# zbw2577/fea-large

Measured on AMD Instinct MI355X. Metric: element-stiffness assemblies/sec, higher is better.
Workload: dtype f64; 1 GPU; 10349856 TET4/1GP neohookean block (66x396x66 Kuhn cubes on the 1x6x1 bar), stiffness+residual assembly, deformed state k1=1.1; elements=10349856, nodes=1782133, scalar_nnz=236453589, clock_ramp_launches_before_warmup=80

## Files before the change

fea-large_amd/csrc/feahip_internal.h:

```cpp
#pragma once
#include <hip/hip_runtime.h>
#include <algorithm>
#include <cstdint>
#include <cstdio>
#include <functional>
#include <initializer_list>
#include <string>
#include <thread>
#include <type_traits>
#include <vector>
#include "../../include/fea_hip.h"

hipError_t feahip_device_malloc(void **p, size_t bytes);
#define hipMalloc(p, bytes) feahip_device_malloc((void **)(p), (bytes))

#define FEA_MAX_NPE 10
#define FEA_MAX_GAUSS 27

#define FEA_CHUNK_BLOCKS 128
#define FEA_CHUNK_ROWS 16
#define FEA_WAVES_PER_WG 4
#define FEA_RED_BLOCKS 2048

struct ElemTable {
// ... 202 lines not shown
#ifndef FEA_Q_SLOTS
#define FEA_Q_SLOTS 5
#endif
#define FEA_Q_REGW 4
#define FEA_Q_MAX_PASS 7
#define FEA_Q_FLANES 128
#define FEA_Q_ROWS_U16 200
struct Gather10Header {
  int r0, r1, b0, nb;
  int nnode, nelem, ntask, npass;
  int nft, fdw;
  unsigned char prow[8];
  unsigned char cnt[40];
  unsigned char sw[8];
  int pad[8];
};
static_assert(FEA_Q_SLOTS * FEA_Q_WAVES <= 40 && FEA_Q_SLOTS <= 8, "Gather10Header: cnt / sw too small");
static_assert(sizeof(Gather10Header) == 128, "Gather10Header is 128 bytes");
struct Gather10Layout {
  int stride;
  int o_nodes, o_elems, o_rows, o_tpos, o_flist, o_clist;
  int max_nodes, max_elems, max_cw, max_fdw, tile_blocks;
};
enum Gather10Limit {
  G10_FITS = FEAHIP_G10_LIMIT_NONE, G10_ELEMS = FEAHIP_G10_LIMIT_ELEMS, G10_ROW_LENGTH = FEAHIP_G10_LIMIT_ROW_LENGTH,
  G10_TASKS = FEAHIP_G10_LIMIT_TASKS, G10_RESIDUAL_LANES = FEAHIP_G10_LIMIT_RESIDUAL_LANES,
  G10_LIST_LENGTH = FEAHIP_G10_LIMIT_LIST_LENGTH, G10_PASSES = FEAHIP_G10_LIMIT_PASSES, G10_OTHER = FEAHIP_G10_LIMIT_OTHER
};
struct HostGather10 : HostChunkMaps {
  Gather10Layout lay;
  std::vector<int> elist;
  int npe = 10;
  int limit = G10_FITS;
  int limit_row = -1;
  int tile_blocks = 0;
};
void build_host_gather10(int N, int E, int npe, const int *conn, const HostPattern &hp, int row_lo, int row_hi, HostGather10 &out);
int ensure_gather10(feahip_ctx *c);
int launch_assemble_gather10(feahip_ctx *c, bool doK, bool doF);

int launch_assemble_visit(feahip_ctx *c, bool doK, bool doF);

enum class MapOutcome { none, built, failed, declined };
struct MapCache {
  int key0 = -1, key1 = -1;
  MapOutcome outcome = MapOutcome::none;
  long long bytes = 0;
  bool built() const { return outcome == MapOutcome::built; }
  bool is(MapOutcome o, int k0, int k1) const { return outcome == o && key0 == k0 && key1 == k1; }
  bool settled(int k0, int k1) const { return is(MapOutcome::built, k0, k1) || is(MapOutcome::failed, k0, k1); }
  void record(MapOutcome o, int k0, int k1) { outcome = o; key0 = k0; key1 = k1; }
};
inline void dev_free(std::initializer_list<void *> ptrs) { for (void *p : ptrs) if (p) (void)hipFree(p); }
struct GenericMaps : MapCache {
  int *d_incptr = nullptr;
  uint32_t *d_inc = nullptr;
  uint8_t *d_incslot = nullptr;
  void release() { dev_free({d_incptr, d_inc, d_incslot}); *this = GenericMaps(); }
};
struct VisitMaps : MapCache {
  VisitDesc *d_desc = nullptr;
  int *d_node = nullptr;
  uint32_t *d_rec = nullptr;
  int nrecords = 0;
  void release() { dev_free({d_desc, d_node, d_rec}); *this = VisitMaps(); }
};
struct QuadMaps : MapCache {
  QuadDesc *d_desc = nullptr;
  uint32_t *d_elem = nullptr, *d_pair = nullptr;
  int *d_node = nullptr;
  int nchunks = 0;
  void release() { dev_free({d_desc, d_elem, d_pair, d_node}); *this = QuadMaps(); }
};
struct GatherCache : MapCache {
  unsigned char *d_maps = nullptr;
  int nchunks = 0;
  double evals_per_element = 0;
  int same_words = 0;
};
struct GatherMaps : GatherCache {
  GatherLayout lay{};
  int *d_run_start = nullptr;
  int nruns = 0;
  std::vector<int> record_of;
  void release() { dev_free({d_maps, d_run_start}); *this = GatherMaps(); }
};
struct Gather10Maps : GatherCache {
  Gather10Layout lay{};
  int *d_elist = nullptr;
  double *d_state = nullptr;
  int nloc = 0;
  void release() { dev_free({d_maps, d_elist, d_state}); *this = Gather10Maps(); }
};

struct SurfaceLoads {
  int nfaces = 0, npf = 0;
  std::vector<int> h_lnode;
  int *d_fnode = nullptr;
  int *d_kind = nullptr;
  double *d_val = nullptr;
  double *d_fc = nullptr;
  int *d_lnode = nullptr, *d_lptr = nullptr, *d_lslot = nullptr;
  void release() { dev_free({d_fnode, d_kind, d_val, d_fc, d_lnode, d_lptr, d_lslot}); *this = SurfaceLoads(); }
};

#define FEA_SURF_MAX_PTS 6
#define FEA_SURF_MAX_NPF 6
struct FaceRule {
  int npt;
  double w[FEA_SURF_MAX_PTS];
  double N[FEA_SURF_MAX_PTS][FEA_SURF_MAX_NPF];
  double dN[FEA_SURF_MAX_PTS][2][FEA_SURF_MAX_NPF];
};
void face_rule(int npf, FaceRule &R);

struct ContactObstacles {
  int n;
  int kind[FEAHIP_MAX_OBSTACLES];
  double c[FEAHIP_MAX_OBSTACLES][3];
  double a[FEAHIP_MAX_OBSTACLES][3];
  double r[FEAHIP_MAX_OBSTACLES];
};
struct ContactState {
  bool set = false;
  int n = 0, nobs = 0;
  double penalty = 0, gap_tolerance = 0;
  int augment_max = 0;
  int kind[FEAHIP_MAX_OBSTACLES] = {0};
  double geom[FEAHIP_MAX_OBSTACLES][10] = {{0}};
  std::vector<int> h_node;
  std::vector<double> h_w;
  int *d_node = nullptr;
  double *d_w = nullptr;
  double *d_mu = nullptr;
  double *d_part = nullptr;
  void release() { dev_free({d_node, d_w, d_mu, d_part}); *this = ContactState(); }
};

struct MassState {
  bool set = false;
  bool stale = false;
  int n_rho = 0, n_mat = 0, Gm = 0;
  std::vector<double> rho, w, N, dN;
  double *d_m_base = nullptr;
  double *d_m = nullptr;
  long long kb0 = -1, kb1 = -1;
  double *d_vel = nullptr, *d_acc = nullptr, *d_xt = nullptr, *d_vt = nullptr;
  double *d_body = nullptr;
  double body[3] = {0, 0, 0};
  double time = 0;
  double *d_ml = nullptr;
  int ml_row0 = -1, ml_row1 = -1;
  double *d_ke_part = nullptr;
  int ke_parts = 0;
  void release_m() { dev_free({d_m_base}); d_m_base = d_m = nullptr; kb0 = kb1 = -1; }
  void release_lump() { dev_free({d_ml, d_ke_part}); d_ml = d_ke_part = nullptr; ml_row0 = ml_row1 = -1; ke_parts = 0; }
  void release() { dev_free({d_m_base, d_vel, d_acc, d_xt, d_vt, d_body, d_ml, d_ke_part}); *this = MassState(); }
};

struct DampingState {
  double alpha = 0, beta = 0;
  double *d_Kd_alloc = nullptr;
  double *d_Kd_base = nullptr;
  double *d_Kd = nullptr;
  int row0 = -1, row1 = -1;
  bool on() const { return alpha > 0.0 || beta > 0.0; }
// ... 525 lines not shown
```

fea-large_amd/csrc/gather_device.h:

```cpp
#pragma once
#include "fem_device.h"
#define PRIO_STATE 0
#define PRIO_GATHER 1
#define PRIO_OUT 3
#include <algorithm>
#include <cstdlib>
#include <cstring>

struct GatherArgs {
  int chunk0, nchunks, model;
  double lambda, mu;
  const ElemTable *tab;
  const unsigned char *maps;
  GatherLayout lay;
  const double *X0, *x;
  double *K, *f;
  int *bad;
  unsigned long long *stamps;
  int ablate;
  const double2 *mat;
};
#if defined(FEAHIP_DEBUG) && !defined(FEAHIP_NOABL)
#define G_ABL(bit) (A.ablate & (bit))
#else
#define G_ABL(bit) 0
#endif

#ifdef FEAHIP_DEBUG
#define G_STAMP(i) do { if (A.stamps) st[i] = __builtin_amdgcn_s_memtime(); } while (0)
#else
#define G_STAMP(i) do { } while (0)
#endif

#define G_RS 0
#define G_RD 66
#define G_VF 130
#define G_SLOT(w) ((w) & 1023u)
#define G_LA(w) (((w) >> 10) & 3)
#define G_LB(w) (((w) >> 12) & 3)

#define GREC 26
#define GREC_F 12

struct GRead { double2 pa, za, pb, qb, zb, vv; };
__device__ __forceinline__ GRead g_fetch(const double *sT, unsigned w)
{
  const double2 *T = reinterpret_cast<const double2 *>(sT + G_SLOT(w) * GREC);
  const int la = G_LA(w), lb = G_LB(w);
  GRead r;
  r.pa = T[la]; r.za = T[8 + la]; r.pb = T[lb]; r.qb = T[4 + lb]; r.zb = T[8 + lb]; r.vv = T[12];
  return r;
}
__device__ __forceinline__ void g_apply(const GRead &r, double (&acc)[9], double &accd)
{
  const double ga0 = r.pa.x, ga1 = r.pa.y, ga2 = r.za.x;
  const double gb0 = r.pb.x, gb1 = r.pb.y, gb2 = r.zb.x;
  const double tb0 = r.qb.x, tb1 = r.qb.y, tb2 = r.zb.y;
  const double vl = r.vv.x, vm = r.vv.y;
  const double h0 = vl * gb0, h1 = vl * gb1, h2 = vl * gb2;
  const double m0 = vm * gb0, m1 = vm * gb1, m2 = vm * gb2;
  accd = fma(ga0, tb0, fma(ga1, tb1, fma(ga2, tb2, accd)));
  acc[0] = fma(ga0, h0, fma(ga0, m0, acc[0])); acc[1] = fma(ga0, h1, fma(ga1, m0, acc[1])); acc[2] = fma(ga0, h2, fma(ga2, m0, acc[2]));
  acc[3] = fma(ga1, h0, fma(ga0, m1, acc[3])); acc[4] = fma(ga1, h1, fma(ga1, m1, acc[4])); acc[5] = fma(ga1, h2, fma(ga2, m1, acc[5]));
  acc[6] = fma(ga2, h0, fma(ga0, m2, acc[6])); acc[7] = fma(ga2, h1, fma(ga1, m2, acc[7])); acc[8] = fma(ga2, h2, fma(ga2, m2, acc[8]));
}
__device__ __forceinline__ void g_finish(double (&acc)[9], double accd)
{
  acc[0] += accd; acc[4] += accd; acc[8] += accd;
}
__device__ __forceinline__ void g_consume(const double *sT, unsigned w, double (&acc)[9], double &accd)
{
  g_apply(g_fetch(sT, w), acc, accd);
}
__device__ __forceinline__ void g_apply_cheap(const GRead &r, double (&acc)[9])
{
  acc[0] += r.pa.x; acc[1] += r.za.x; acc[2] += r.pb.x; acc[3] += r.qb.x; acc[4] += r.zb.x; acc[5] += r.vv.x;
}
__device__ __forceinline__ GRead g_fetch_cheap(const double *sT, unsigned w)
{
  GRead r; const double v = (double)w;
  r.pa = make_double2(v, v); r.za = r.pa; r.pb = r.pa; r.qb = r.pa; r.zb = r.pa; r.vv = r.pa;
  return r;
}
// ... 181 lines not shown
    for (int b = 0; b < 4; ++b)
#pragma unroll
      for (int i = 0; i < 3; ++i) R[b * 3 + i] = g[b][i];
    const double T00 = S[0][0] + vm, T11 = S[1][1] + vm, T22 = S[2][2] + vm;
#pragma unroll
    for (int b = 0; b < 4; ++b) {
      R[12 + b * 3 + 0] = fma(T00, g[b][0], fma(S[0][1], g[b][1], S[0][2] * g[b][2]));
      R[12 + b * 3 + 1] = fma(T11, g[b][1], fma(S[0][1], g[b][0], S[1][2] * g[b][2]));
      R[12 + b * 3 + 2] = fma(T22, g[b][2], fma(S[0][2], g[b][0], S[1][2] * g[b][1]));
    }
    R[24] = vd * lambda;
    R[25] = vm;
  } else {
#pragma unroll
    for (int b = 1; b < 4; ++b)
#pragma unroll
      for (int i = 0; i < 3; ++i) R[b * 3 + i] = S[i][0] * g[b][0] + S[i][1] * g[b][1] + S[i][2] * g[b][2];
#pragma unroll
    for (int i = 0; i < 3; ++i) R[i] = -((R[3 + i] + R[6 + i]) + R[9 + i]);
  }
  return detJ;
}

template <int CTRL>
__device__ __forceinline__ double g_quad_perm(double x)
{
  int lo = __double2loint(x), hi = __double2hiint(x);
  lo = __builtin_amdgcn_update_dpp(0, lo, CTRL, 0xF, 0xF, true);
  hi = __builtin_amdgcn_update_dpp(0, hi, CTRL, 0xF, 0xF, true);
  return __hiloint2double(hi, lo);
}
__device__ __forceinline__ double g_quad_sum(double v)
{
  v += g_quad_perm<0xB1>(v);
  v += g_quad_perm<0x4E>(v);
  return v;
}

#define G_BARRIER() do { __builtin_amdgcn_fence(__ATOMIC_RELEASE, "workgroup", "local"); __builtin_amdgcn_s_barrier(); \
                         __builtin_amdgcn_fence(__ATOMIC_ACQUIRE, "workgroup", "local"); } while (0)

typedef int g_v8i __attribute__((ext_vector_type(8)));
typedef int g_v4i __attribute__((ext_vector_type(4)));

struct GMaps {
  unsigned eids, tpos, cw[FEA_G_REGW], vw[2];
  int kd, vb, ve;
};

#define G_TASK_THREADS FEA_G_TASK_THREADS

template <bool DOK, bool DOF>
__device__ __forceinline__ void g_load_maps(const GatherLayout &lay, const unsigned char *rec, int t, GMaps &m)
{
  const unsigned short *rows = reinterpret_cast<const unsigned short *>(rec + lay.o_rows);
  m.eids = 0xFFFFFFFFu; m.tpos = 0; m.kd = m.vb = m.ve = 0;
#pragma unroll
  for (int k = 0; k < FEA_G_REGW; ++k) m.cw[k] = 0;
  m.vw[0] = m.vw[1] = 0;
  if (t < lay.max_elems) m.eids = reinterpret_cast<const unsigned *>(rec + lay.o_elems)[t];
  if (DOK && t < ((lay.max_tasks + 63) & ~63)) {
    m.tpos = reinterpret_cast<const unsigned *>(rec + lay.o_bpos)[t];
#pragma unroll
    for (int k = 0; k < FEA_G_REGW; ++k)
      if (k < lay.max_depth) m.cw[k] = reinterpret_cast<const unsigned *>(rec + lay.o_clist)[k * FEA_G_THREADS + t];
  }
  if (DOK && t >= G_TASK_THREADS) {
    const int l = t - G_TASK_THREADS;
    m.kd = rows[G_RD + (l >> 2)];
#pragma unroll
    for (int k = 0; k < FEA_G_REGW; ++k)
      if (k < lay.max_ddepth) m.cw[k] = reinterpret_cast<const unsigned *>(rec + lay.o_dlist)[k * FEA_G_DIAG_LANES + l];
  }
  if (!DOK && t < ((lay.max_vthr + 63) & ~63)) {
#pragma unroll
    for (int v = 0; v < 2; ++v)
      if (v < lay.max_vdepth) m.vw[v] = reinterpret_cast<const unsigned short *>(rec + lay.o_vlist)[v * FEA_G_THREADS + t];
  }
  if (!DOK) {
    const int fr = min(t / 3, FEA_G_MAX_ROWS - 1);
    m.vb = rows[G_VF + fr]; m.ve = rows[G_VF + fr + 1];
  }
}
```

fea-large_amd/csrc/kernels_gather.hip:

```cpp
#include "gather_device.h"
#ifndef G_NT_ROWS
#define G_NT_ROWS 1
#endif
template <bool DOK, bool DOF, bool NH, bool HET>
__global__ __launch_bounds__(FEA_G_THREADS, FEA_G_BIG ? 4 : 3)
void k_assemble_gather(GatherArgs A, const int *__restrict__ run_start, int nruns)
{
  extern __shared__ double2 g_smem[];
  double2 *sC = g_smem;
  double *sT = reinterpret_cast<double *>(g_smem + A.lay.max_nodes * 3);
  const int t = threadIdx.x;
#ifdef FEAHIP_DEBUG
  unsigned long long st[8] = {0, 0, 0, 0, 0, 0, 0, 0}, sa[8] = {0, 0, 0, 0, 0, 0, 0, 0};
  const unsigned long long clk0 = __builtin_amdgcn_s_memtime(), real0 = __builtin_amdgcn_s_memrealtime();
#endif
  const int per = ((int)gridDim.x + 7) >> 3;
  const int ridx = ((int)blockIdx.x & 7) * per + ((int)blockIdx.x >> 3);
  if (ridx >= nruns) return;
  int chunk = run_start[ridx];
  const int cend = run_start[ridx + 1];
  if (chunk >= cend) return;
  constexpr int REC = DOK ? GREC : GREC_F;
  const size_t stride = (size_t)A.lay.stride;
  const unsigned char *rec = A.maps + (size_t)(A.chunk0 + chunk) * stride;
  const bool node_lane = t < A.lay.max_nodes;
  const int wslot = __builtin_amdgcn_readfirstlane(t >> 6);

  const double gauss_w = A.tab->w[0];
  GMaps mn;
  g_load_maps<DOK, DOF>(A.lay, G_ABL(64) ? A.maps + (size_t)A.chunk0 * stride : rec, t, mn);
  GatherHeader hn = *reinterpret_cast<const GatherHeader *>(rec);
  int node1 = reinterpret_cast<const int *>(rec + A.lay.o_nodes)[t & (FEA_G_MAX_NODES - 1)];
  if (node_lane) {
    const double *gx = A.x + (size_t)node1 * 4, *gX = A.X0 + (size_t)node1 * 4;
    const double2 a0 = *reinterpret_cast<const double2 *>(gx), a1 = *reinterpret_cast<const double2 *>(gx + 2);
    const double2 c0 = *reinterpret_cast<const double2 *>(gX), c1 = *reinterpret_cast<const double2 *>(gX + 2);
    sC[t * 3] = a0; sC[t * 3 + 1] = make_double2(a1.x, c0.x); sC[t * 3 + 2] = make_double2(c0.y, c1.x);
  }
  {
    const int cn = min(chunk + 1, cend - 1);
    node1 = reinterpret_cast<const int *>(A.maps + (size_t)(A.chunk0 + cn) * stride + A.lay.o_nodes)[t & (FEA_G_MAX_NODES - 1)];
  }
  int mid1 = 0;
  double2 pn = make_double2(A.lambda, A.mu);
  if constexpr (HET) {
    pn = A.mat[rec[A.lay.o_emat + t]];
    const int cn = min(chunk + 1, cend - 1);
    mid1 = (A.maps + (size_t)(A.chunk0 + cn) * stride + A.lay.o_emat)[t];
    asm volatile("" : : "v"(mid1), "v"(pn.x), "v"(pn.y));
  }
  asm volatile("" : : "v"(mn.eids), "v"(mn.tpos), "v"(mn.cw[0]), "v"(mn.cw[1]), "v"(mn.cw[2]), "v"(mn.cw[3]), "v"(mn.cw[4]), "v"(mn.cw[5]),
               "v"(mn.vw[0]), "v"(mn.vw[1]), "v"(mn.kd), "v"(mn.vb), "v"(mn.ve), "v"(node1), "v"(gauss_w));
  G_BARRIER();

  for (;;) {
    G_STAMP(0);
    const bool more = chunk + 1 < cend;
    const GatherHeader h = hn;
    int hword;
    double2 ca0, ca1, cc0, cc1;
    const GMaps m = mn;
    const int nrows = h.r1 - h.r0;
    const unsigned wdw = wslot < 4 ? h.wdepth[0] : (wslot < 8 ? h.wdepth[1] : h.wdepth[2]);
    const int wd = wslot < G_TASK_THREADS / 64 ? (int)((wdw >> (8 * (wslot & 3))) & 255u) : 0;
    rec = A.maps + (size_t)(A.chunk0 + chunk) * stride;

    __builtin_amdgcn_s_setprio(PRIO_STATE);
    if (t < h.nelem && m.eids != 0xFFFFFFFFu) {
      const unsigned eids = m.eids;
      const int nd[4] = {(int)(eids & 255u), (int)((eids >> 8) & 255u), (int)((eids >> 16) & 255u), (int)(eids >> 24)};
      double xe[4][3], Xe[4][3];
#pragma unroll
      for (int k = 0; k < 4; ++k) {
        const double2 *cc = sC + nd[k] * 3;
        const double2 p0 = cc[0], p1 = cc[1], p2 = cc[2];
        xe[k][0] = p0.x; xe[k][1] = p0.y; xe[k][2] = p1.x;
        Xe[k][0] = p1.y; Xe[k][1] = p2.x; Xe[k][2] = p2.y;
      }
      double R[REC];
      double detJ;
      if (G_ABL(8)) { detJ = 1.0; for (int q = 0; q < REC; ++q) R[q] = xe[q & 3][q % 3] + Xe[(q >> 2) & 3][q % 3]; }
      else detJ = NH ? lintet_record_nh<DOK>(xe, Xe, gauss_w, HET ? pn.x : A.lambda, HET ? pn.y : A.mu, R)
                     : lintet_record_a5<DOK>(xe, Xe, gauss_w, HET ? pn.x : A.lambda, HET ? pn.y : A.mu, R);
      if (!(detJ > 0.0)) {
        if (DOK) {
          const int *gn = reinterpret_cast<const int *>(rec + A.lay.o_nodes);
          const int g0 = min(min(gn[nd[0]], gn[nd[1]]), min(gn[nd[2]], gn[nd[3]]));
          if (g0 >= h.r0 && g0 < h.r1) atomicAdd(A.bad, 1);
        }
      }
      if (detJ == 0.0) {
        double2 *o = reinterpret_cast<double2 *>(sT + t * REC);
#pragma unroll
        for (int q = 0; q < REC / 2; ++q) o[q] = make_double2(0.0, 0.0);
      } else if (!G_ABL(1)) g_store_record<DOK>(sT + t * REC, R);
      else sT[t * REC] = R[0] + R[25 % REC];
    } else if (t < h.nelem) {
      double2 *o = reinterpret_cast<double2 *>(sT + t * REC);
#pragma unroll
      for (int q = 0; q < REC / 2; ++q) o[q] = make_double2(0.0, 0.0);
    }
    {
      const int c1 = min(chunk + 1, cend - 1), c2 = min(chunk + 2, cend - 1);
      const unsigned char *rec1 = A.maps + (size_t)(A.chunk0 + c1) * stride;
      hword = reinterpret_cast<const int *>(rec1)[t & 15];
      if (!(h.flags & 1) || G_ABL(64)) g_load_maps<DOK, DOF>(A.lay, G_ABL(64) ? A.maps + (size_t)A.chunk0 * stride : rec1, t, mn);
      if (wslot < FEA_G_MAX_NODES / 64) {
        const size_t n1 = (size_t)(node_lane ? node1 : 0);
        ca0 = *reinterpret_cast<const double2 *>(A.x + n1 * 4); ca1.x = A.x[n1 * 4 + 2];
        cc0 = *reinterpret_cast<const double2 *>(A.X0 + n1 * 4); cc1.x = A.X0[n1 * 4 + 2];
        node1 = reinterpret_cast<const int *>(A.maps + (size_t)(A.chunk0 + c2) * stride + A.lay.o_nodes)[t & (FEA_G_MAX_NODES - 1)];
      }
      if constexpr (HET) {
        if (wslot * 64 < A.lay.max_elems) {
          pn = A.mat[mid1];
          mid1 = (A.maps + (size_t)(A.chunk0 + c2) * stride + A.lay.o_emat)[t];
        }
      }
    }

    G_LDS_DRAIN();
    G_BARRIER();
    G_STAMP(1);

    __builtin_amdgcn_s_setprio(PRIO_GATHER);
    double acc[9] = {0, 0, 0, 0, 0, 0, 0, 0, 0}, accd = 0;
    if (DOK && t < h.noffd) {
#define G_FETCH(w) (G_ABL(4) ? g_fetch_cheap(sT, w) : g_fetch(sT, w))
#define G_APPLY(r) do { if (G_ABL(2)) g_apply_cheap(r, acc); else g_apply(r, acc, accd); } while (0)
#pragma unroll
      for (int k = 0; k < FEA_G_REGW; ++k)
        if (k < wd) { { const GRead r = G_FETCH(m.cw[k] & 0xFFFFu); G_APPLY(r); } { const GRead r = G_FETCH(m.cw[k] >> 16); G_APPLY(r); } }
      for (int k = FEA_G_REGW; k < wd; ++k) {
        const unsigned w = reinterpret_cast<const unsigned *>(rec + A.lay.o_clist)[k * FEA_G_THREADS + t];
        g_consume(sT, w & 0xFFFFu, acc, accd); g_consume(sT, w >> 16, acc, accd);
      }
      g_finish(acc, accd);
    }
    double dg[6] = {0, 0, 0, 0, 0, 0};
    double fa[3] = {0, 0, 0};
    if (DOK && t >= G_TASK_THREADS && t - G_TASK_THREADS < 4 * nrows) {
#pragma unroll
      for (int k = 0; k < FEA_G_REGW; ++k)
        if (k < h.ddepth) { g_consume_diag<DOF>(sT, m.cw[k] & 0xFFFFu, dg, fa); g_consume_diag<DOF>(sT, m.cw[k] >> 16, dg, fa); }
      for (int k = FEA_G_REGW; k < h.ddepth; ++k) {
        const unsigned w = reinterpret_cast<const unsigned *>(rec + A.lay.o_dlist)[k * FEA_G_DIAG_LANES + t - G_TASK_THREADS];
        g_consume_diag<DOF>(sT, w & 0xFFFFu, dg, fa); g_consume_diag<DOF>(sT, w >> 16, dg, fa);
      }
    }
    if (!DOK && t < h.nvthr) {
      g_visit<DOK>(sT, m.vw[0], fa);
      if (h.vdepth > 1) g_visit<DOK>(sT, m.vw[1], fa);
      for (int v = 2; v < h.vdepth; ++v)
        g_visit<DOK>(sT, reinterpret_cast<const unsigned short *>(rec + A.lay.o_vlist)[v * FEA_G_THREADS + t], fa);
    }
    G_STAMP(2);
    __builtin_amdgcn_s_setprio(PRIO_OUT);
    G_BARRIER();
    G_STAMP(3);

    const int odd = h.b0 & 1;
    double *sK = sT + odd;
    double *sF = DOK ? sT + ((A.lay.max_tile * 9 + 3) & ~1) : sT;
    if (DOK && t < h.noffd && !G_ABL(16)) {
      const int bpos = (int)(m.tpos & 0xFFFFu), mpos = (int)(m.tpos >> 16);
      if (bpos != 0xFFFF) {
#pragma unroll
        for (int q = 0; q < 9; ++q) sK[bpos * 9 + q] = acc[q];
      }
      if (mpos != 0xFFFF) {
#pragma unroll
        for (int i = 0; i < 3; ++i)
#pragma unroll
          for (int j = 0; j < 3; ++j) sK[mpos * 9 + 3 * j + i] = acc[3 * i + j];
      }
    }
    if (DOK && t >= G_TASK_THREADS) {
#pragma unroll
      for (int q = 0; q < 6; ++q) dg[q] = g_quad_sum(dg[q]);
      if (DOF) {
#pragma unroll
        for (int q = 0; q < 3; ++q) fa[q] = g_quad_sum(fa[q]);
      }
      if ((t & 3) == 0 && t - G_TASK_THREADS < 4 * nrows) {
        double *o = sK + m.kd * 9;
        o[0] = dg[0]; o[1] = dg[1]; o[2] = dg[2]; o[3] = dg[1]; o[4] = dg[3]; o[5] = dg[4]; o[6] = dg[2]; o[7] = dg[4]; o[8] = dg[5];
      }
    }
    if (!DOK && t < h.nvthr) { sF[t * 3] = fa[0]; sF[t * 3 + 1] = fa[1]; sF[t * 3 + 2] = fa[2]; }
    G_STAMP(4);
    asm volatile("" : : "v"(mn.eids), "v"(mn.tpos), "v"(mn.cw[0]), "v"(mn.cw[1]), "v"(mn.cw[2]), "v"(mn.cw[3]), "v"(mn.cw[4]), "v"(mn.cw[5]),
                 "v"(mn.vw[0]), "v"(mn.vw[1]), "v"(mn.kd), "v"(mn.vb), "v"(mn.ve), "v"(node1), "v"(hword));
    if constexpr (HET) asm volatile("" : : "v"(mid1), "v"(pn.x), "v"(pn.y));
    if (more && node_lane) {
      sC[t * 3] = ca0; sC[t * 3 + 1] = make_double2(ca1.x, cc0.x); sC[t * 3 + 2] = make_double2(cc0.y, cc1.x);
    }
    hn.r0 = __builtin_amdgcn_readlane(hword, 0); hn.r1 = __builtin_amdgcn_readlane(hword, 1);
    hn.b0 = __builtin_amdgcn_readlane(hword, 2); hn.nb = __builtin_amdgcn_readlane(hword, 3);
    hn.nnode = __builtin_amdgcn_readlane(hword, 4); hn.nelem = __builtin_amdgcn_readlane(hword, 5);
    hn.noffd = __builtin_amdgcn_readlane(hword, 6); hn.depth = __builtin_amdgcn_readlane(hword, 7);
    hn.nvthr = __builtin_amdgcn_readlane(hword, 8); hn.vdepth = __builtin_amdgcn_readlane(hword, 9);
    hn.ddepth = __builtin_amdgcn_readlane(hword, 10);
    hn.wdepth[0] = (unsigned)__builtin_amdgcn_readlane(hword, 11); hn.wdepth[1] = (unsigned)__builtin_amdgcn_readlane(hword, 12);
    hn.wdepth[2] = (unsigned)__builtin_amdgcn_readlane(hword, 13); hn.flags = __builtin_amdgcn_readlane(hword, 14);
    G_BARRIER();
    G_STAMP(5);
    if (!DOK) {
      const int ft = t;
      const int fr = ft / 3, fi = ft - 3 * fr;
      if (fr < nrows) {
        double a = 0;
        for (int k = m.vb; k < m.ve; ++k) a += sF[k * 3 + fi];
        A.f[(size_t)(h.r0 + fr) * 3 + fi] = a;
      }
    }
    if (DOK && DOF && t >= G_TASK_THREADS && (t & 3) == 0 && t - G_TASK_THREADS < 4 * nrows) {
      double *fo = A.f + (size_t)(h.r0 + ((t - G_TASK_THREADS) >> 2)) * 3;
      fo[0] = fa[0]; fo[1] = fa[1]; fo[2] = fa[2];
    }
    if (DOK) {
      double *Kd = A.K + (size_t)h.b0 * 9;
      const int total = h.nb * 9;
      if (odd && t == 0) Kd[0] = sK[0];
      const int npair = (total - odd) >> 1;
      for (int j = t; j < npair; j += FEA_G_THREADS) {
        const int p = odd + 2 * j;
        if (G_ABL(32) && j >= 64) break;
#if G_NT_ROWS
        __builtin_nontemporal_store(*reinterpret_cast<const g_v2d *>(sK + p), reinterpret_cast<g_v2d *>(Kd + p));
#else
        *reinterpret_cast<double2 *>(Kd + p) = *reinterpret_cast<const double2 *>(sK + p);
#endif
      }
      if (((total - odd) & 1) && t == 0) Kd[total - 1] = sK[total - 1];
    }
    G_BARRIER();
    G_STAMP(6);
#ifdef FEAHIP_DEBUG
    if (A.stamps) for (int i = 0; i < 6; ++i) sa[i] += st[i + 1] - st[i];
#endif
    if (!more) break;
    ++chunk;
  }
#ifdef FEAHIP_DEBUG
  if (A.stamps && (t & 63) == 0) {
    unsigned long long *o = A.stamps + ((size_t)ridx * (FEA_G_THREADS / 64) + (t >> 6)) * 8;
    for (int i = 0; i < 6; ++i) o[i] = sa[i];
    o[6] = __builtin_amdgcn_s_memtime() - clk0;
    o[7] = __builtin_amdgcn_s_memrealtime() - real0;
  }
#endif
}

static int device_cus(int device)
{
  static int ncu_of[64];
  int &ncu = ncu_of[device & 63];
  if (ncu <= 0) { hipDeviceProp_t p; ncu = (hipGetDeviceProperties(&p, device) == hipSuccess && p.multiProcessorCount > 0) ? p.multiProcessorCount : 256; }
  return ncu;
}

int ensure_gather(feahip_ctx *c)
{
  GatherMaps &g = c->gather;
  if (g.settled(c->row0, c->row1)) return FEAHIP_OK;
  if (!c->h_pat || c->h_conn.empty() || !c->linear_tet || c->G != 1) return FEAHIP_OK;
  g.release();
  HostGather hg;
  build_host_gather(c->N, c->E, c->h_conn.data(), *c->h_pat, c->row0, c->row1, hg, c->n_materials ? c->h_elem_mat.data() : nullptr,
                    device_cus(c->device));
  if (!hg.ok) { g.record(MapOutcome::failed, c->row0, c->row1); return FEAHIP_OK; }
  FEA_HIP_CHECK(c, hipMalloc((void **)&g.d_maps, hg.blob.size() ? hg.blob.size() : 1));
  FEA_HIP_CHECK(c, hipMemcpy(g.d_maps, hg.blob.data(), hg.blob.size(), hipMemcpyHostToDevice));
  g.nruns = (int)hg.run_start.size() - 1;
  FEA_HIP_CHECK(c, hipMalloc((void **)&g.d_run_start, sizeof(int) * hg.run_start.size()));
  FEA_HIP_CHECK(c, hipMemcpy(g.d_run_start, hg.run_start.data(), sizeof(int) * hg.run_start.size(), hipMemcpyHostToDevice));
  g.record_of.assign((size_t)hg.nchunks, 0);
  for (int i = 0; i < hg.nchunks; ++i) g.record_of[hg.walk[i]] = i;
  g.lay = hg.lay;
  g.nchunks = hg.nchunks;
  g.bytes = (long long)hg.blob.size();
  g.evals_per_element = hg.distinct_elems ? (double)hg.total_evals / (double)hg.distinct_elems : 0.0;
  g.same_words = hg.same_as_previous;
  g.record(MapOutcome::built, c->row0, c->row1);
  return FEAHIP_OK;
}

#ifdef FEAHIP_DEBUG
extern "C" int feahip_debug_gather_record(feahip_ctx *c, int chunk, int *layout_ints, unsigned char *record)
{
  int rc = ensure_gather(c);
  const GatherMaps &g = c->gather;
  if (rc || !g.built()) return FEAHIP_ESTATE;
  if (chunk < 0) chunk = g.nchunks / 2;
  if (chunk >= g.nchunks) return FEAHIP_EINVAL;
  memcpy(layout_ints, &g.lay, sizeof(GatherLayout));
  if (record) (void)hipMemcpy(record, g.d_maps + (size_t)g.record_of[chunk] * g.lay.stride, g.lay.stride, hipMemcpyDeviceToHost);
  return (int)(sizeof(GatherLayout) / sizeof(int));
}
#endif

int launch_assemble_gather(feahip_ctx *c, bool doK, bool doF)
{
  const GatherMaps &g = c->gather;
  GatherArgs A;
  A.chunk0 = 0; A.nchunks = g.nchunks; A.model = c->model; A.lambda = c->lambda; A.mu = c->mu;
  A.tab = c->d_table; A.maps = g.d_maps; A.lay = g.lay; A.X0 = c->d_X0; A.x = c->d_x;
  A.K = c->d_K; A.f = c->d_f; A.bad = c->d_flag + 1; A.stamps = nullptr; A.ablate = 0; A.mat = c->d_mat;
  if (g.nchunks <= 0) return FEAHIP_OK;
#ifdef FEAHIP_DEBUG
  static unsigned long long *d_stamps = nullptr;
  static int stamps_cap = 0;
  { const char *e = getenv("FEAHIP_GATHER_ABLATE"); A.ablate = e ? atoi(e) : 0; }
  const char *dbg = getenv("FEAHIP_GATHER_STAMPS");
  if (dbg && atoi(dbg)) {
    if (!d_stamps || stamps_cap < g.nchunks) {
      if (d_stamps) (void)hipFree(d_stamps);
      (void)hipMalloc((void **)&d_stamps, sizeof(unsigned long long) * 8 * (FEA_G_THREADS / 64) * (size_t)g.nchunks);
      (void)hipMemset(d_stamps, 0, sizeof(unsigned long long) * 8 * (FEA_G_THREADS / 64) * (size_t)g.nchunks);
      stamps_cap = g.nchunks;
    }
    A.stamps = d_stamps;
  }
#endif
  const int nruns = g.nruns;
  const dim3 grid((nruns + 7) & ~7), blk(FEA_G_THREADS);
  const int regK = std::max(A.lay.max_elems * GREC, ((A.lay.max_tile * 9 + 3) & ~1) + 3 * FEA_G_THREADS);
  const int regF = std::max(A.lay.max_elems * GREC_F, 3 * FEA_G_THREADS);
  const int ldsK = A.lay.max_nodes * 48 + ((regK + 1) & ~1) * 8, ldsF = A.lay.max_nodes * 48 + ((regF + 1) & ~1) * 8;
  const bool nh = c->model == FEAHIP_MODEL_COMPRESSIBLE_NEOHOOKEAN;
  const bool het = c->n_materials > 0;
  if (het != (g.lay.o_emat != 0)) { c->err = "gather maps and material table disagree"; return FEAHIP_ESTATE; }
  if (het && !nh && doK && !doF) {
    if (!c->d_f_discard) FEA_HIP_CHECK(c, hipMalloc((void **)&c->d_f_discard, sizeof(double) * (size_t)c->ndof));
    A.f = c->d_f_discard;
    doF = true;
  }
  auto launch = [&](auto K, auto F, auto M, auto H) -> int {
    if constexpr (H && K && !F && !M) { c->err = "gather assembly: no K-only A5 kernel with a material table"; return FEAHIP_ESTATE; }
    else {
    const int lds = K ? ldsK : ldsF;
    FEA_HIP_CHECK(c, hipFuncSetAttribute(reinterpret_cast<const void *>(&k_assemble_gather<K, F, M, H>), hipFuncAttributeMaxDynamicSharedMemorySize, lds));
    hipLaunchKernelGGL((k_assemble_gather<K, F, M, H>), grid, blk, lds, c->stream, A, g.d_run_start, nruns);
    return FEAHIP_OK;
    }
  };
  int rc;
  with_kf(doK, doF, [&](auto K, auto F) {
    auto model = [&](auto H) { return nh ? launch(K, F, std::true_type(), H) : launch(K, F, std::false_type(), H); };
    rc = het ? model(std::true_type()) : model(std::false_type());
  });
  if (rc) return rc;
  FEA_HIP_CHECK(c, hipGetLastError());
#ifdef FEAHIP_DEBUG
  if (A.stamps) {
    static int calls = 0;
    if (++calls == 50) {
      (void)hipStreamSynchronize(c->stream);
      constexpr int NW = FEA_G_THREADS / 64;
      std::vector<unsigned long long> hst((size_t)g.nchunks * 8 * NW);
      (void)hipMemcpy(hst.data(), A.stamps, hst.size() * 8, hipMemcpyDeviceToHost);
      double sum[NW][8] = {};
      for (int i = 0; i < nruns; ++i)
        for (int w = 0; w < NW; ++w)
          for (int q = 0; q < 8; ++q) sum[w][q] += (double)hst[((size_t)i * NW + w) * 8 + q];
      fprintf(stderr, "[gather stamps] in-kernel clock %.0f MHz (s_memtime / s_memrealtime x 100 MHz over a run), run = %.0f shader cycles, %d runs of %d chunks\n",
              sum[0][7] > 0 ? 100.0 * sum[0][6] / sum[0][7] : 0.0, sum[0][6] / nruns, nruns, g.nchunks);
      if (const char *path = getenv("FEAHIP_GATHER_STAMPS_FILE")) {
        if (FILE *fo = fopen(path, "wb")) {
          const long long head[2] = {nruns, NW};
          fwrite(head, sizeof(head), 1, fo);
          fwrite(hst.data(), sizeof(unsigned long long), (size_t)nruns * NW * 8, fo);
          fclose(fo);
        }
      }
      for (int w = 0; w < NW; w += (NW > 4 ? 5 : 1))
        fprintf(stderr, "[gather stamps K=%d F=%d wave %d, per chunk] state %.0f  gather %.0f  barrier B %.0f  tile writes %.0f  wait for the prefetched words + coordinates + barrier C %.0f  rows out (+ barrier D) %.0f cycles\n",
                (int)doK, (int)doF, w, sum[w][0] / g.nchunks, sum[w][1] / g.nchunks, sum[w][2] / g.nchunks, sum[w][3] / g.nchunks,
                sum[w][4] / g.nchunks, sum[w][5] / g.nchunks);
    }
  }
#endif
  return FEAHIP_OK;
}
```

Before: 16.69 billion elements/s.

## Stage the K tile write-out so global row stores overlap LDS tile writes

For the K-assembling gather kernels, the LDS tile write and the global row streaming are split into NS stages (default 4). Each stage writes its slice of blocks into shared memory, then streams the previous slice to global memory, with a barrier between stages, so global stores can start before the whole tile is written. The trade is extra block-wide barriers and per-stage range checks on every thread. An environment variable can restore the single-stage path, and debug stamps are extended to time each stage.

```diff
diff --git a/fea-large_amd/csrc/feahip_internal.h b/fea-large_amd/csrc/feahip_internal.h
--- a/fea-large_amd/csrc/feahip_internal.h
+++ b/fea-large_amd/csrc/feahip_internal.h
@@ -308,6 +308,7 @@
   GatherLayout lay{};
   int *d_run_start = nullptr;
   int nruns = 0;
+  int stages = 0;
   std::vector<int> record_of;
   void release() { dev_free({d_maps, d_run_start}); *this = GatherMaps(); }
 };
diff --git a/fea-large_amd/csrc/gather_device.h b/fea-large_amd/csrc/gather_device.h
--- a/fea-large_amd/csrc/gather_device.h
+++ b/fea-large_amd/csrc/gather_device.h
@@ -1,4 +1,22 @@
 #pragma once
+#if defined(__HIPCC__) || defined(__CUDACC__)
+#define G_HD __host__ __device__
+#else
+#define G_HD
+#endif
+struct GStage { int b0, b1, j0, j1; };
+G_HD inline int g_stage_cut(int nb, int ns, int s) { return (int)(((unsigned)s * (unsigned)nb + (unsigned)ns - 1u) / (unsigned)ns); }
+G_HD inline int g_stage_pairs_below(int b, int odd) { const int d = 9 * b - odd; return d > 0 ? d >> 1 : 0; }
+G_HD inline GStage g_stage(int nb, int odd, int ns, int s)
+{
+  GStage g;
+  g.b0 = g_stage_cut(nb, ns, s); g.b1 = g_stage_cut(nb, ns, s + 1);
+  g.j0 = g_stage_pairs_below(g.b0, odd); g.j1 = g_stage_pairs_below(g.b1, odd);
+  return g;
+}
+G_HD inline bool g_stream_front(int nb, int odd) { return odd && nb > 0; }
+G_HD inline bool g_stream_back(int nb, int odd) { return nb > 0 && ((9 * nb - odd) & 1); }
+#ifndef GATHER_STAGES_ONLY
 #include "fem_device.h"
 #define PRIO_STATE 0
 #define PRIO_GATHER 1
@@ -346,3 +364,4 @@
     m.vb = rows[G_VF + fr]; m.ve = rows[G_VF + fr + 1];
   }
 }
+#endif
diff --git a/fea-large_amd/csrc/kernels_gather.hip b/fea-large_amd/csrc/kernels_gather.hip
--- a/fea-large_amd/csrc/kernels_gather.hip
+++ b/fea-large_amd/csrc/kernels_gather.hip
@@ -2,16 +2,22 @@
 #ifndef G_NT_ROWS
 #define G_NT_ROWS 1
 #endif
-template <bool DOK, bool DOF, bool NH, bool HET>
+#ifndef G_STAGES
+#define G_STAGES 4
+#endif
+template <bool DOK, bool DOF, bool NH, bool HET, int NS>
 __global__ __launch_bounds__(FEA_G_THREADS, FEA_G_BIG ? 4 : 3)
 void k_assemble_gather(GatherArgs A, const int *__restrict__ run_start, int nruns)
 {
+  static_assert(NS >= 1 && (DOK || NS == 1), "stages of the write-out: the kernels that assemble K only");
   extern __shared__ double2 g_smem[];
   double2 *sC = g_smem;
   double *sT = reinterpret_cast<double *>(g_smem + A.lay.max_nodes * 3);
   const int t = threadIdx.x;
 #ifdef FEAHIP_DEBUG
   unsigned long long st[8] = {0, 0, 0, 0, 0, 0, 0, 0}, sa[8] = {0, 0, 0, 0, 0, 0, 0, 0};
+  unsigned long long sb[8] = {0, 0, 0, 0, 0, 0, 0, 0};
+  static_assert(NS <= 7, "one stamp slot per stage, the last one for the wait for the prefetched words");
   const unsigned long long clk0 = __builtin_amdgcn_s_memtime(), real0 = __builtin_amdgcn_s_memrealtime();
 #endif
   const int per = ((int)gridDim.x + 7) >> 3;
@@ -159,6 +165,7 @@
     G_BARRIER();
     G_STAMP(3);
 
+    if constexpr (NS == 1) {
     const int odd = h.b0 & 1;
     double *sK = sT + odd;
     double *sF = DOK ? sT + ((A.lay.max_tile * 9 + 3) & ~1) : sT;
@@ -192,6 +199,7 @@
     asm volatile("" : : "v"(mn.eids), "v"(mn.tpos), "v"(mn.cw[0]), "v"(mn.cw[1]), "v"(mn.cw[2]), "v"(mn.cw[3]), "v"(mn.cw[4]), "v"(mn.cw[5]),
                  "v"(mn.vw[0]), "v"(mn.vw[1]), "v"(mn.kd), "v"(mn.vb), "v"(mn.ve), "v"(node1), "v"(hword));
     if constexpr (HET) asm volatile("" : : "v"(mid1), "v"(pn.x), "v"(pn.y));
+    G_STAMP(7);
     if (more && node_lane) {
       sC[t * 3] = ca0; sC[t * 3 + 1] = make_double2(ca1.x, cc0.x); sC[t * 3 + 2] = make_double2(cc0.y, cc1.x);
     }
@@ -234,10 +242,104 @@
       }
       if (((total - odd) & 1) && t == 0) Kd[total - 1] = sK[total - 1];
     }
+    } else {
+      const int odd = h.b0 & 1;
+      double *sK = sT + odd;
+      const int bpos = (int)(m.tpos & 0xFFFFu), mpos = (int)(m.tpos >> 16);
+      const bool block_thread = t < h.noffd;
+      const bool diag_lane = t >= G_TASK_THREADS && (t & 3) == 0 && t - G_TASK_THREADS < 4 * nrows;
+      auto tile_blocks = [&](const GStage &g) {
+        if (block_thread) {
+          if (bpos >= g.b0 && bpos < g.b1) {
+#pragma unroll
+            for (int q = 0; q < 9; ++q) sK[bpos * 9 + q] = acc[q];
+          }
+          if (mpos >= g.b0 && mpos < g.b1) {
+#pragma unroll
+            for (int i = 0; i < 3; ++i)
+#pragma unroll
+              for (int j = 0; j < 3; ++j) sK[mpos * 9 + 3 * j + i] = acc[3 * i + j];
+          }
+        }
+      };
+      auto tile_diag = [&](const GStage &g) {
+        if (diag_lane && m.kd >= g.b0 && m.kd < g.b1) {
+          double *o = sK + m.kd * 9;
+          o[0] = dg[0]; o[1] = dg[1]; o[2] = dg[2]; o[3] = dg[1]; o[4] = dg[3]; o[5] = dg[4]; o[6] = dg[2]; o[7] = dg[4]; o[8] = dg[5];
+        }
+      };
+      double *Kd = A.K + (size_t)h.b0 * 9;
+      auto rows = [&](const GStage &g) {
+        for (int j = g.j0 + t; j < g.j1; j += FEA_G_THREADS) {
+          const int p = odd + 2 * j;
+#if G_NT_ROWS
+          __builtin_nontemporal_store(*reinterpret_cast<const g_v2d *>(sK + p), reinterpret_cast<g_v2d *>(Kd + p));
+#else
+          *reinterpret_cast<double2 *>(Kd + p) = *reinterpret_cast<const double2 *>(sK + p);
+#endif
+        }
+      };
+      const GStage g0 = g_stage(h.nb, odd, NS, 0);
+      tile_blocks(g0);
+      if (t >= G_TASK_THREADS) {
+#pragma unroll
+        for (int q = 0; q < 6; ++q) dg[q] = g_quad_sum(dg[q]);
+        if (DOF) {
+#pragma unroll
+          for (int q = 0; q < 3; ++q) fa[q] = g_quad_sum(fa[q]);
+        }
+      }
+      tile_diag(g0);
+      G_STAMP(4);
+      asm volatile("" : : "v"(mn.eids), "v"(mn.tpos), "v"(mn.cw[0]), "v"(mn.cw[1]), "v"(mn.cw[2]), "v"(mn.cw[3]), "v"(mn.cw[4]), "v"(mn.cw[5]),
+                   "v"(mn.vw[0]), "v"(mn.vw[1]), "v"(mn.kd), "v"(mn.vb), "v"(mn.ve), "v"(node1), "v"(hword));
+      if constexpr (HET) asm volatile("" : : "v"(mid1), "v"(pn.x), "v"(pn.y));
+      G_STAMP(7);
+      if (more && node_lane) {
+        sC[t * 3] = ca0; sC[t * 3 + 1] = make_double2(ca1.x, cc0.x); sC[t * 3 + 2] = make_double2(cc0.y, cc1.x);
+      }
+      hn.r0 = __builtin_amdgcn_readlane(hword, 0); hn.r1 = __builtin_amdgcn_readlane(hword, 1);
+      hn.b0 = __builtin_amdgcn_readlane(hword, 2); hn.nb = __builtin_amdgcn_readlane(hword, 3);
+      hn.nnode = __builtin_amdgcn_readlane(hword, 4); hn.nelem = __builtin_amdgcn_readlane(hword, 5);
+      hn.noffd = __builtin_amdgcn_readlane(hword, 6); hn.depth = __builtin_amdgcn_readlane(hword, 7);
+      hn.nvthr = __builtin_amdgcn_readlane(hword, 8); hn.vdepth = __builtin_amdgcn_readlane(hword, 9);
+      hn.ddepth = __builtin_amdgcn_readlane(hword, 10);
+      hn.wdepth[0] = (unsigned)__builtin_amdgcn_readlane(hword, 11); hn.wdepth[1] = (unsigned)__builtin_amdgcn_readlane(hword, 12);
+      hn.wdepth[2] = (unsigned)__builtin_amdgcn_readlane(hword, 13); hn.flags = __builtin_amdgcn_readlane(hword, 14);
+      G_BARRIER();
+      G_STAMP(5);
+#ifdef FEAHIP_DEBUG
+      unsigned long long sg = st[5];
+#endif
+      if (DOF && diag_lane) {
+        double *fo = A.f + (size_t)(h.r0 + ((t - G_TASK_THREADS) >> 2)) * 3;
+        fo[0] = fa[0]; fo[1] = fa[1]; fo[2] = fa[2];
+      }
+      if (g_stream_front(h.nb, odd) && t == 0) Kd[0] = sK[0];
+#pragma unroll
+      for (int s = 0; s < NS; ++s) {
+        rows(s == 0 ? g0 : g_stage(h.nb, odd, NS, s));
+        if (s + 1 < NS) {
+          const GStage gn = g_stage(h.nb, odd, NS, s + 1);
+          tile_blocks(gn);
+          tile_diag(gn);
+          G_BARRIER();
+#ifdef FEAHIP_DEBUG
+          if (A.stamps) { const unsigned long long now = __builtin_amdgcn_s_memtime(); sb[s] += now - sg; sg = now; }
+#endif
+        }
+      }
+      if (g_stream_back(h.nb, odd) && t == 0) Kd[h.nb * 9 - 1] = sK[h.nb * 9 - 1];
+#ifdef FEAHIP_DEBUG
+      if (A.stamps) sb[NS - 1] -= sg;
+#endif
+    }
     G_BARRIER();
     G_STAMP(6);
 #ifdef FEAHIP_DEBUG
     if (A.stamps) for (int i = 0; i < 6; ++i) sa[i] += st[i + 1] - st[i];
+    if (NS > 1 && A.stamps) sb[NS - 1] += st[6];
+    if (A.stamps) sb[7] += st[7] - st[4];
 #endif
     if (!more) break;
     ++chunk;
@@ -248,6 +350,10 @@
     for (int i = 0; i < 6; ++i) o[i] = sa[i];
     o[6] = __builtin_amdgcn_s_memtime() - clk0;
     o[7] = __builtin_amdgcn_s_memrealtime() - real0;
+    {
+      unsigned long long *o2 = o + (size_t)nruns * (FEA_G_THREADS / 64) * 8;
+      for (int i = 0; i < 8; ++i) o2[i] = sb[i];
+    }
   }
 #endif
 }
@@ -282,6 +388,7 @@
   g.bytes = (long long)hg.blob.size();
   g.evals_per_element = hg.distinct_elems ? (double)hg.total_evals / (double)hg.distinct_elems : 0.0;
   g.same_words = hg.same_as_previous;
+  { const char *e = getenv("FEAHIP_GATHER_STAGES"); g.stages = e && atoi(e) == 1 ? 1 : G_STAGES; }
   g.record(MapOutcome::built, c->row0, c->row1);
   return FEAHIP_OK;
 }
@@ -316,8 +423,8 @@
   if (dbg && atoi(dbg)) {
     if (!d_stamps || stamps_cap < g.nchunks) {
       if (d_stamps) (void)hipFree(d_stamps);
-      (void)hipMalloc((void **)&d_stamps, sizeof(unsigned long long) * 8 * (FEA_G_THREADS / 64) * (size_t)g.nchunks);
-      (void)hipMemset(d_stamps, 0, sizeof(unsigned long long) * 8 * (FEA_G_THREADS / 64) * (size_t)g.nchunks);
+      (void)hipMalloc((void **)&d_stamps, sizeof(unsigned long long) * 16 * (FEA_G_THREADS / 64) * (size_t)g.nchunks);
+      (void)hipMemset(d_stamps, 0, sizeof(unsigned long long) * 16 * (FEA_G_THREADS / 64) * (size_t)g.nchunks);
       stamps_cap = g.nchunks;
     }
     A.stamps = d_stamps;
@@ -336,18 +443,22 @@
     A.f = c->d_f_discard;
     doF = true;
   }
-  auto launch = [&](auto K, auto F, auto M, auto H) -> int {
+  auto launch = [&](auto K, auto F, auto M, auto H, auto S) -> int {
     if constexpr (H && K && !F && !M) { c->err = "gather assembly: no K-only A5 kernel with a material table"; return FEAHIP_ESTATE; }
     else {
+    constexpr int NS = K ? (int)S : 1;
     const int lds = K ? ldsK : ldsF;
-    FEA_HIP_CHECK(c, hipFuncSetAttribute(reinterpret_cast<const void *>(&k_assemble_gather<K, F, M, H>), hipFuncAttributeMaxDynamicSharedMemorySize, lds));
-    hipLaunchKernelGGL((k_assemble_gather<K, F, M, H>), grid, blk, lds, c->stream, A, g.d_run_start, nruns);
+    FEA_HIP_CHECK(c, hipFuncSetAttribute(reinterpret_cast<const void *>(&k_assemble_gather<K, F, M, H, NS>), hipFuncAttributeMaxDynamicSharedMemorySize, lds));
+    hipLaunchKernelGGL((k_assemble_gather<K, F, M, H, NS>), grid, blk, lds, c->stream, A, g.d_run_start, nruns);
     return FEAHIP_OK;
     }
   };
   int rc;
   with_kf(doK, doF, [&](auto K, auto F) {
-    auto model = [&](auto H) { return nh ? launch(K, F, std::true_type(), H) : launch(K, F, std::false_type(), H); };
+    auto stages = [&](auto M, auto H) {
+      return g.stages == 1 ? launch(K, F, M, H, std::integral_constant<int, 1>()) : launch(K, F, M, H, std::integral_constant<int, G_STAGES>());
+    };
+    auto model = [&](auto H) { return nh ? stages(std::true_type(), H) : stages(std::false_type(), H); };
     rc = het ? model(std::true_type()) : model(std::false_type());
   });
   if (rc) return rc;
@@ -358,7 +469,7 @@
     if (++calls == 50) {
       (void)hipStreamSynchronize(c->stream);
       constexpr int NW = FEA_G_THREADS / 64;
-      std::vector<unsigned long long> hst((size_t)g.nchunks * 8 * NW);
+      std::vector<unsigned long long> hst((size_t)g.nchunks * 16 * NW);
       (void)hipMemcpy(hst.data(), A.stamps, hst.size() * 8, hipMemcpyDeviceToHost);
       double sum[NW][8] = {};
       for (int i = 0; i < nruns; ++i)
@@ -378,6 +489,21 @@
         fprintf(stderr, "[gather stamps K=%d F=%d wave %d, per chunk] state %.0f  gather %.0f  barrier B %.0f  tile writes %.0f  wait for the prefetched words + coordinates + barrier C %.0f  rows out (+ barrier D) %.0f cycles\n",
                 (int)doK, (int)doF, w, sum[w][0] / g.nchunks, sum[w][1] / g.nchunks, sum[w][2] / g.nchunks, sum[w][3] / g.nchunks,
                 sum[w][4] / g.nchunks, sum[w][5] / g.nchunks);
+      if (doK) {
+        const int ns = g.stages == 1 ? 1 : G_STAGES;
+        const unsigned long long *h2 = hst.data() + (size_t)nruns * NW * 8;
+        for (int w = 0; w < NW; w += (NW > 4 ? 5 : 1)) {
+          double sg[8] = {};
+          for (int i = 0; i < nruns; ++i)
+            for (int q = 0; q < 8; ++q) sg[q] += (double)h2[((size_t)i * NW + w) * 8 + q];
+          fprintf(stderr, "[gather stamps K=%d F=%d wave %d, per chunk] of the wait + coordinates + barrier C: the wait for the prefetched words %.0f cycles\n",
+                  (int)doK, (int)doF, w, sg[7] / g.nchunks);
+          if (ns == 1) continue;
+          fprintf(stderr, "[gather stamps K=%d F=%d wave %d, per chunk] %d stages: W(0) %.0f ", (int)doK, (int)doF, w, ns, sum[w][3] / g.nchunks);
+          for (int q = 0; q + 1 < ns; ++q) fprintf(stderr, " { R(%d) ; W(%d) ; barrier } %.0f ", q, q + 1, sg[q] / g.nchunks);
+          fprintf(stderr, " R(%d) + barrier D %.0f cycles\n", ns - 1, sg[ns - 1] / g.nchunks);
+        }
+      }
     }
   }
 #endif
```

Result: slower. 14.48 billion elements/s (-13.3%).
